# dash-robotics/perception

Measured on AMD Instinct MI355X. Metric: frames/sec (640x480 D435 cloud, plane+cluster+ICP), higher is better.
Workload: dtype f32

## Files before the change

### perception_amd/csrc/k_icp_lat.hip

```cpp
#include "kernels.hpp"
#include "icp_solve_row.hpp"
#include "lat_search.hpp"

namespace cd {

#ifdef CD_LAT_TIMERS
__device__ unsigned long long g_lat_stats[8];
extern "C" int cd_debug_lat_stats(unsigned long long* out, int reset) {
    if (hipMemcpyFromSymbol(out, HIP_SYMBOL(g_lat_stats), sizeof(g_lat_stats)) != hipSuccess) return -1;
    if (reset) { unsigned long long z[8] = {0}; (void)hipMemcpyToSymbol(HIP_SYMBOL(g_lat_stats), z, sizeof(z)); }
    return 0;
}
#define LAT_T(k) { const long long tn_ = clock64(); tph[k] += tn_ - tlast; tlast = tn_; }
#else
#define LAT_T(k)
#endif

struct LatSlot {
    int k, src_off, n, tslot;
    int phase;
    int gen;
    int ready;
    int pad;
};
enum { LAT_ITER = 0, LAT_FIT = 1, LAT_EMPTY = 2 };

#ifndef CD_LAT_SOLVE_ROW
#define CD_LAT_SOLVE_ROW 1
#endif
#ifndef CD_LAT_WAVES_PER_EU
#define CD_LAT_WAVES_PER_EU 4
#endif
template <int CPW, int WPC, bool BOUNDED>
__global__ void __launch_bounds__(CPW * WPC * WAVE, CD_LAT_WAVES_PER_EU)
k_icp_lat(int nitems, const int* __restrict__ order, const IcpCluster* __restrict__ cl, IcpState* __restrict__ st,
          unsigned long long* __restrict__ accf, const IcpLattice* __restrict__ lats, float4* __restrict__ src,
          const float4* __restrict__ src0, int* __restrict__ queue, unsigned long long* __restrict__ busy,
          unsigned long long* __restrict__ busy_out, IcpParams prm, IcpBound bnd) {
    __shared__ float4 s_tab[CPW][LAT_MAX_TAB];
    __shared__ int4 s_face[CPW][2 * LAT_MAX_FACES];
    __shared__ unsigned long long s_acc[CPW][16];
    __shared__ IcpState s_so[CPW];
    __shared__ LatSlot s_slot[CPW];
    __shared__ int s_flags[2];
    __shared__ unsigned s_nv[BOUNDED ? CPW : 1];
    const int lane = threadIdx.x & 63, wave = threadIdx.x >> 6;
    const int slot = wave / WPC, sub = wave % WPC;
    const long long wg_t0 = wall_clock64();
    auto refill = [&](int s) {
        LatSlot& sl = s_slot[s];
        for (int i = 0; i < 16; ++i) s_acc[s][i] = 0ull;
        if constexpr (BOUNDED) s_nv[s] = 0u;
        sl.ready = 0;
        for (;;) {
            const int item = atomicAdd(queue, 1);
            if (item >= nitems) { sl.phase = LAT_EMPTY; return; }
            const int k = order[item];
            if (st[2 * (size_t)k].done) continue;
            const IcpCluster c = cl[k];
            sl.k = k; sl.src_off = c.src_off; sl.n = c.n; sl.tslot = c.slot;
            s_so[s] = st[2 * (size_t)k];
            sl.phase = LAT_ITER;
            sl.gen += 1;
            return;
        }
    };
    if (threadIdx.x < CPW) { s_slot[threadIdx.x].gen = 0; refill(threadIdx.x); }
    if (threadIdx.x == 0) { s_flags[0] = 0; s_flags[1] = 1; }
    __syncthreads();
    int my_gen = 0;
#ifdef CD_LAT_TIMERS
    long long tph[6] = {0, 0, 0, 0, 0, 0}, tlast = clock64();
#endif
    for (;;) {
        if (s_flags[1]) {
            const LatSlot sl = s_slot[slot];
            const bool mine = sl.phase != LAT_EMPTY && sl.gen != my_gen;
            if (mine) {
                const IcpLattice* __restrict__ L = lats + sl.tslot;
                for (int i = sub * WAVE + lane; i < L->ntab; i += WPC * WAVE) s_tab[slot][i] = L->tab[i];
                if (sub == 0 && lane < LAT_MAX_FACES) {
                    const int f = lane, w = L->w[f], u = L->fast[f], v = 3 - w - u;
                    s_face[slot][f] = make_int4(w, u, L->base[f], __float_as_int(L->c[f]));
                    s_face[slot][LAT_MAX_FACES + f] = make_int4(L->toff[u], L->toff[v < 0 || v > 2 ? 0 : v], L->n[u], 0);
                }
                my_gen = sl.gen;
            }
            __syncthreads();
        }
        LAT_T(5)
        {
            const int phase = __builtin_amdgcn_readfirstlane(s_slot[slot].phase), n = __builtin_amdgcn_readfirstlane(s_slot[slot].n);
            const int src_off = __builtin_amdgcn_readfirstlane(s_slot[slot].src_off), tslot = __builtin_amdgcn_readfirstlane(s_slot[slot].tslot);
            const int npass = (n + 63) >> 6;
            float4* pts = src + src_off;
            const float4* tab = s_tab[slot];
            const int4* face = s_face[slot];
            LatFaces F;
            {
                const IcpLattice* __restrict__ L = lats + (phase == LAT_EMPTY ? 0 : tslot);
                lat_faces_load(L, F);
            }
            const bool nf3 = F.nface <= 3;
            if (phase == LAT_ITER) {
                const bool moved = s_so[slot].iters > 0;
                float T[12];
#pragma unroll
                for (int i = 0; i < 12; ++i) T[i] = s_so[slot].T[i];
                unsigned long long S[16];
#pragma unroll
                for (int i = 0; i < 16; ++i) S[i] = 0ull;
                unsigned nv = 0u;
                float4 pnext = pts[min((sub << 6) + lane, n - 1)];
                for (int pss = sub; pss < npass; pss += WPC) {
                    const int myq = (pss << 6) + lane;
                    const bool act = myq < n;
                    const float4 p = pnext;
                    pnext = pts[min(((pss + WPC) << 6) + lane, n - 1)];
                    float px = p.x, py = p.y, pz = p.z;
                    if (moved) {
                        xform(T, p.x, p.y, p.z, px, py, pz);
                        if (act) pts[myq] = make_float4(px, py, pz, p.w);
                    }
                    const LatHit h = F.axes ? lat_nearest_axes<true>(tab, face, F, px, py, pz)
                                            : (nf3 ? lat_nearest<true, 3>(tab, face, F, px, py, pz) : lat_nearest<true, LAT_MAX_FACES>(tab, face, F, px, py, pz));
                    const bool keep = act && (!BOUNDED || h.d <= bnd.d2_max);
                    if constexpr (BOUNDED) nv += (unsigned)__popcll(ballot64(keep));
                    if (keep) {
                        const float pv[3] = {px, py, pz}, qv[3] = {h.nx, h.ny, h.nz};
                        const float big_c = fmaxf(fmaxf(fmaxf(fabsf(px), fabsf(py)), fabsf(pz)), fmaxf(fmaxf(fabsf(h.nx), fabsf(h.ny)), fabsf(h.nz)));
                        if (big_c < 256.f && h.d < 16384.f) {
#pragma unroll
                            for (int a = 0; a < 3; ++a) {
                                S[a] += LatFix<FIX_SHIFT>::bits(pv[a]);
                                S[3 + a] += LatFix<FIX_SHIFT>::bits(qv[a]);
#pragma unroll
                                for (int b = 0; b < 3; ++b) S[6 + 3 * a + b] += LatFix<FIX_SHIFT>::bits(__fmul_rn(qv[a], pv[b]));
                            }
                            S[15] += LatFix<FIX_SHIFT_D2>::bits(h.d);
                        } else {
#pragma unroll
                            for (int a = 0; a < 3; ++a) {
                                S[a] += (unsigned long long)fixq(pv[a], FIX_SHIFT) + LatFix<FIX_SHIFT>::C;
                                S[3 + a] += (unsigned long long)fixq(qv[a], FIX_SHIFT) + LatFix<FIX_SHIFT>::C;
#pragma unroll
                                for (int b = 0; b < 3; ++b) S[6 + 3 * a + b] += (unsigned long long)fixq(__fmul_rn(qv[a], pv[b]), FIX_SHIFT) + LatFix<FIX_SHIFT>::C;
                            }
                            S[15] += (unsigned long long)fixq(h.d, FIX_SHIFT_D2) + LatFix<FIX_SHIFT_D2>::C;
                        }
                    }
                }
                if (sub < npass) wave_fold_to_lds(S, 16, s_acc[slot]);
                if constexpr (BOUNDED) { if (sub < npass && lane == 0) atomicAdd(&s_nv[slot], nv); }
                if (sub == 0 && lane == 0) s_slot[slot].ready = 1;
            } else if (phase == LAT_FIT) {
                const float4* pts0 = src0 + src_off;
                float T[12], Tf[12];
#pragma unroll
                for (int i = 0; i < 12; ++i) {
                    T[i] = __int_as_float(__builtin_amdgcn_readfirstlane(__float_as_int(s_so[slot].T[i])));
                    Tf[i] = __int_as_float(__builtin_amdgcn_readfirstlane(__float_as_int(s_so[slot].Tfinal[i])));
                }
                unsigned long long S[16];
#pragma unroll
                for (int i = 0; i < 16; ++i) S[i] = 0ull;
                float4 pnext = pts[min((sub << 6) + lane, n - 1)], p0next = pts0[min((sub << 6) + lane, n - 1)];
                for (int pss = sub; pss < npass; pss += WPC) {
                    const int myq = (pss << 6) + lane;
                    const bool act = myq < n;
                    const float4 p = pnext, p0 = p0next;
                    pnext = pts[min(((pss + WPC) << 6) + lane, n - 1)];
                    p0next = pts0[min(((pss + WPC) << 6) + lane, n - 1)];
                    float ox, oy, oz;
                    xform(T, p.x, p.y, p.z, ox, oy, oz);
                    if (act) pts[myq] = make_float4(ox, oy, oz, p.w);
                    float qx, qy, qz;
                    xform(Tf, p0.x, p0.y, p0.z, qx, qy, qz);
                    const LatHit h = F.axes ? lat_nearest_axes<false>(tab, face, F, qx, qy, qz)
                                            : (nf3 ? lat_nearest<false, 3>(tab, face, F, qx, qy, qz) : lat_nearest<false, LAT_MAX_FACES>(tab, face, F, qx, qy, qz));
                    if (act) S[0] += h.d < 16384.f ? LatFix<FIX_SHIFT_D2>::bits(h.d) : (unsigned long long)fixq(h.d, FIX_SHIFT_D2) + LatFix<FIX_SHIFT_D2>::C;
                }
                if (sub < npass) wave_fold_to_lds(S, 1, s_acc[slot]);
            }
        }
        LAT_T(0)
        if (threadIdx.x == 0) s_flags[1] = 0;
        __syncthreads();
        LAT_T(1)
#if CD_LAT_SOLVE_ROW
        const int tid = (int)threadIdx.x | s_flags[0];
        if (tid < CPW * 16) {
            const int s = tid >> 4, l = tid & 15;
            LatSlot& sl = s_slot[s];
            const int phase = sl.phase, ready = sl.ready;
            const int nv = BOUNDED && phase == LAT_ITER ? (int)s_nv[s] : sl.n;
            const unsigned long long off = (unsigned long long)nv * LatFix<FIX_SHIFT>::C, off_d = (unsigned long long)nv * LatFix<FIX_SHIFT_D2>::C;
            if (phase == LAT_ITER && ready) {
                RowLanes row(tid);
                RowLanes::V<unsigned long long> a;
                a.v = s_acc[s][l] - (l == 15 ? off_d : off);
                const int done = icp_step_row<BOUNDED>(row, s_so[s], a, nv, prm);
                s_acc[s][l] = 0ull;
                if (l == 0) {
                    if (done) sl.phase = LAT_FIT;
                    if constexpr (BOUNDED) s_nv[s] = 0u;
                    sl.ready = 0;
                }
            } else if (phase == LAT_FIT && l == 0) {
                s_so[s].done = 1;
                st[2 * (size_t)sl.k] = s_so[s];
                st[2 * (size_t)sl.k + 1] = s_so[s];
                accf[sl.k] = s_acc[s][0] - off_d;
                refill(s);
                if (sl.phase != LAT_EMPTY) s_flags[1] = 1;
            }
        }
#else
        if (threadIdx.x < CPW) {
            const int s = threadIdx.x;
            LatSlot& sl = s_slot[s];
            const int nv = BOUNDED && sl.phase == LAT_ITER ? (int)s_nv[s] : sl.n;
            const unsigned long long off = (unsigned long long)nv * LatFix<FIX_SHIFT>::C, off_d = (unsigned long long)nv * LatFix<FIX_SHIFT_D2>::C;
            if (sl.phase == LAT_ITER && sl.ready) {
                for (int i = 0; i < 15; ++i) s_acc[s][i] -= off;
                s_acc[s][15] -= off_d;
                if (icp_step<BOUNDED>(s_so[s], s_acc[s], nv, prm)) sl.phase = LAT_FIT;
                for (int i = 0; i < 16; ++i) s_acc[s][i] = 0ull;
                if constexpr (BOUNDED) s_nv[s] = 0u;
                sl.ready = 0;
            } else if (sl.phase == LAT_FIT) {
                s_so[s].done = 1;
                st[2 * (size_t)sl.k] = s_so[s];
                st[2 * (size_t)sl.k + 1] = s_so[s];
                accf[sl.k] = s_acc[s][0] - off_d;
                refill(s);
                if (sl.phase != LAT_EMPTY) s_flags[1] = 1;
            }
        }
#endif
        LAT_T(2)
        __syncthreads();
        LAT_T(3)
#ifdef CD_LAT_TIMERS
        tph[4] += 1;
#endif
        int all_empty = 1;
#pragma unroll
        for (int s = 0; s < CPW; ++s) all_empty &= s_slot[s].phase == LAT_EMPTY ? 1 : 0;
        if (all_empty) break;
    }
#ifdef CD_LAT_TIMERS
    if (threadIdx.x == 0) for (int i = 0; i < 6; ++i) atomicAdd(&g_lat_stats[i], (unsigned long long)tph[i]);
#endif
    if (threadIdx.x == 0 && busy) {
        atomicAdd(busy, (unsigned long long)(wall_clock64() - wg_t0) * (unsigned long long)(CPW * WPC));
        if (busy_out) {
            __threadfence();
            if (atomicAdd(queue + 1, 1) == (int)gridDim.x - 1) {
                __threadfence();
                *busy_out = atomicAdd(busy, 0ull);
            }
        }
    }
}

__device__ __forceinline__ bool lat_same_bits(float a, float b) { return __float_as_uint(a) == __float_as_uint(b); }

__global__ void __launch_bounds__(BLOCK) k_lat_nn(const IcpLattice* __restrict__ L, const float4* __restrict__ q, int n, int* __restrict__ out_idx,
                                                  float* __restrict__ out_d2) {
    __shared__ float4 s_tab[LAT_MAX_TAB];
    __shared__ int4 s_face[2 * LAT_MAX_FACES];
    LatFaces F;
    lat_stage<BLOCK>(L, F, s_tab, s_face);
    for (int base = blockIdx.x * BLOCK; base < n; base += gridDim.x * BLOCK) {
        const int i = base + threadIdx.x;
        const float4 p = q[i < n ? i : n - 1];
        const LatHit h = lat_nearest<true, LAT_MAX_FACES, true>(s_tab, s_face, F, p.x, p.y, p.z);
        const LatHit g = lat_nearest<false, 3>(s_tab, s_face, F, p.x, p.y, p.z);
        bool same = F.nface > 3 || h.d == g.d;
        const int idx = lat_index(s_face, F, h);
        if (F.axes) {
            const LatHit a = lat_nearest_axes<true, true>(s_tab, s_face, F, p.x, p.y, p.z);
            const LatHit b = lat_nearest_axes<false>(s_tab, s_face, F, p.x, p.y, p.z);
            same = same && a.d == h.d && b.d == h.d && lat_same_bits(a.nx, h.nx) && lat_same_bits(a.ny, h.ny) && lat_same_bits(a.nz, h.nz) &&
                   lat_index(s_face, F, a) == idx;
        }
        if (i < n) { out_idx[i] = idx; out_d2[i] = same ? h.d : __uint_as_float(0x7fc00000u); }
    }
}

template <int CPW, int WPC>
static void launch_lat_shape(hipStream_t s, int nitems, int n_wg, const int* order, const IcpCluster* cl, IcpState* st, unsigned long long* accf,
                             const IcpLattice* lats, float4* src, const float4* src0, int* queue, unsigned long long* busy, unsigned long long* busy_out,
                             IcpParams prm, const IcpBound& bnd) {
    if (bnd.bounded)
        hipLaunchKernelGGL((k_icp_lat<CPW, WPC, true>), dim3(n_wg), dim3(CPW * WPC * WAVE), 0, s, nitems, order, cl, st, accf, lats, src, src0, queue, busy, busy_out, prm, bnd);
    else
        hipLaunchKernelGGL((k_icp_lat<CPW, WPC, false>), dim3(n_wg), dim3(CPW * WPC * WAVE), 0, s, nitems, order, cl, st, accf, lats, src, src0, queue, busy, busy_out, prm, bnd);
}
void launch_icp_lat(hipStream_t s, int nitems, int cpw, int wpc, int n_wg, const IcpProblems& P, const IcpTemplates& T, const IcpScratch& S,
                    unsigned long long* busy, unsigned long long* busy_out, IcpParams prm, const IcpBound& bnd) {
    if (nitems <= 0 || n_wg <= 0) return;
#define CD_LAT_CASE(C, W) if (cpw == C && wpc == W) return launch_lat_shape<C, W>(s, nitems, n_wg, P.order, P.cl, P.st, P.accf, T.lats, S.src, S.src0, S.queue, busy, busy_out, prm, bnd);
    CD_LAT_CASE(1, 1) CD_LAT_CASE(1, 2) CD_LAT_CASE(1, 4) CD_LAT_CASE(1, 8) CD_LAT_CASE(1, 16)
    CD_LAT_CASE(2, 1) CD_LAT_CASE(2, 2) CD_LAT_CASE(2, 4)
    CD_LAT_CASE(4, 1) CD_LAT_CASE(4, 2) CD_LAT_CASE(4, 4)
    CD_LAT_CASE(8, 1) CD_LAT_CASE(8, 2)
#undef CD_LAT_CASE
    launch_lat_shape<1, 4>(s, nitems, n_wg, P.order, P.cl, P.st, P.accf, T.lats, S.src, S.src0, S.queue, busy, busy_out, prm, bnd);
}
void launch_lat_nn(hipStream_t s, const IcpLattice* lat, const float4* q, int n, int* out_idx, float* out_d2) {
    if (n <= 0) return;
    const int g = (n + BLOCK - 1) / BLOCK;
    hipLaunchKernelGGL(k_lat_nn, dim3(g < 1024 ? g : 1024), dim3(BLOCK), 0, s, lat, q, n, out_idx, out_d2);
}

}
```

Baseline: 209,500.

## Replace wave reduction of moment sums with DPP row-transpose fold

Replaces the generic wave_fold_to_lds reduction of the 16 fixed-point 64-bit moment sums with a transpose-style fold. Half the lanes swap registers, and DPP adds within a row halve the live sums at each step, so each lane of a 16-lane row ends up holding one distinct sum. permlane16/32 swaps then combine the rows, and each of the first 16 lanes does one LDS atomic. The __syncthreads after the per-slot work is also swapped for a raw lgkmcnt wait plus s_barrier, which skips waiting on outstanding global memory ops. It adds timer probes and a host-side check of the fold, and it relies on hand-written asm DPP and gfx950 permlane intrinsics.

```diff
diff --git a/perception_amd/csrc/k_icp_lat.hip b/perception_amd/csrc/k_icp_lat.hip
--- a/perception_amd/csrc/k_icp_lat.hip
+++ b/perception_amd/csrc/k_icp_lat.hip
@@ -1,19 +1,24 @@
 #include "kernels.hpp"
 #include "icp_solve_row.hpp"
 #include "lat_search.hpp"
+#include "lat_fold.hpp"
 
 namespace cd {
 
 #ifdef CD_LAT_TIMERS
-__device__ unsigned long long g_lat_stats[8];
+__device__ unsigned long long g_lat_stats[16];
 extern "C" int cd_debug_lat_stats(unsigned long long* out, int reset) {
     if (hipMemcpyFromSymbol(out, HIP_SYMBOL(g_lat_stats), sizeof(g_lat_stats)) != hipSuccess) return -1;
-    if (reset) { unsigned long long z[8] = {0}; (void)hipMemcpyToSymbol(HIP_SYMBOL(g_lat_stats), z, sizeof(z)); }
+    if (reset) { unsigned long long z[16] = {0}; (void)hipMemcpyToSymbol(HIP_SYMBOL(g_lat_stats), z, sizeof(z)); }
     return 0;
 }
-#define LAT_T(k) { const long long tn_ = clock64(); tph[k] += tn_ - tlast; tlast = tn_; }
+#define LAT_T(k) { const long long tn_ = clock64(); tph[k] += tn_ - tlast; tlast = tn_; tsub = tn_; }
+#define LAT_S(k) { const long long tn_ = clock64(); tph[k] += tn_ - tsub; tsub = tn_; }
+#define LAT_VM() asm volatile("s_waitcnt vmcnt(0)" ::: "memory");
 #else
 #define LAT_T(k)
+#define LAT_S(k)
+#define LAT_VM()
 #endif
 
 struct LatSlot {
@@ -31,6 +36,8 @@
 #ifndef CD_LAT_WAVES_PER_EU
 #define CD_LAT_WAVES_PER_EU 4
 #endif
+__device__ __forceinline__ void lds_barrier() { asm volatile("s_waitcnt lgkmcnt(0)\n\ts_barrier" ::: "memory"); }
+
 template <int CPW, int WPC, bool BOUNDED>
 __global__ void __launch_bounds__(CPW * WPC * WAVE, CD_LAT_WAVES_PER_EU)
 k_icp_lat(int nitems, const int* __restrict__ order, const IcpCluster* __restrict__ cl, IcpState* __restrict__ st,
@@ -70,7 +77,7 @@
     __syncthreads();
     int my_gen = 0;
 #ifdef CD_LAT_TIMERS
-    long long tph[6] = {0, 0, 0, 0, 0, 0}, tlast = clock64();
+    long long tph[10] = {0, 0, 0, 0, 0, 0, 0, 0, 0, 0}, tlast = clock64(), tsub = tlast;
 #endif
     for (;;) {
         if (s_flags[1]) {
@@ -112,6 +119,7 @@
                 for (int i = 0; i < 16; ++i) S[i] = 0ull;
                 unsigned nv = 0u;
                 float4 pnext = pts[min((sub << 6) + lane, n - 1)];
+                LAT_VM() LAT_S(6)
                 for (int pss = sub; pss < npass; pss += WPC) {
                     const int myq = (pss << 6) + lane;
                     const bool act = myq < n;
@@ -150,9 +158,11 @@
                         }
                     }
                 }
-                if (sub < npass) wave_fold_to_lds(S, 16, s_acc[slot]);
+                LAT_S(7)
+                if (sub < npass) wave_fold_rows_to_lds<16>(S, s_acc[slot]);
                 if constexpr (BOUNDED) { if (sub < npass && lane == 0) atomicAdd(&s_nv[slot], nv); }
                 if (sub == 0 && lane == 0) s_slot[slot].ready = 1;
+                LAT_S(8)
             } else if (phase == LAT_FIT) {
                 const float4* pts0 = src0 + src_off;
                 float T[12], Tf[12];
@@ -165,6 +175,7 @@
 #pragma unroll
                 for (int i = 0; i < 16; ++i) S[i] = 0ull;
                 float4 pnext = pts[min((sub << 6) + lane, n - 1)], p0next = pts0[min((sub << 6) + lane, n - 1)];
+                LAT_VM() LAT_S(6)
                 for (int pss = sub; pss < npass; pss += WPC) {
                     const int myq = (pss << 6) + lane;
                     const bool act = myq < n;
@@ -180,12 +191,14 @@
                                             : (nf3 ? lat_nearest<false, 3>(tab, face, F, qx, qy, qz) : lat_nearest<false, LAT_MAX_FACES>(tab, face, F, qx, qy, qz));
                     if (act) S[0] += h.d < 16384.f ? LatFix<FIX_SHIFT_D2>::bits(h.d) : (unsigned long long)fixq(h.d, FIX_SHIFT_D2) + LatFix<FIX_SHIFT_D2>::C;
                 }
-                if (sub < npass) wave_fold_to_lds(S, 1, s_acc[slot]);
+                LAT_S(7)
+                if (sub < npass) wave_fold_rows_to_lds<1>(S, s_acc[slot]);
+                LAT_S(8)
             }
         }
         LAT_T(0)
         if (threadIdx.x == 0) s_flags[1] = 0;
-        __syncthreads();
+        lds_barrier();
         LAT_T(1)
 #if CD_LAT_SOLVE_ROW
         const int tid = (int)threadIdx.x | s_flags[0];
@@ -250,7 +263,7 @@
         if (all_empty) break;
     }
 #ifdef CD_LAT_TIMERS
-    if (threadIdx.x == 0) for (int i = 0; i < 6; ++i) atomicAdd(&g_lat_stats[i], (unsigned long long)tph[i]);
+    if (threadIdx.x == 0) for (int i = 0; i < 10; ++i) atomicAdd(&g_lat_stats[i], (unsigned long long)tph[i]);
 #endif
     if (threadIdx.x == 0 && busy) {
         atomicAdd(busy, (unsigned long long)(wall_clock64() - wg_t0) * (unsigned long long)(CPW * WPC));
diff --git a/perception_amd/csrc/lat_fold.hpp b/perception_amd/csrc/lat_fold.hpp
--- /dev/null
+++ b/perception_amd/csrc/lat_fold.hpp
@@ -0,0 +1,104 @@
+#pragma once
+
+#ifdef __HIPCC__
+#define CD_FOLD_FN __device__ __forceinline__
+#else
+#define CD_FOLD_FN inline
+#endif
+
+namespace cd {
+
+enum { LANE_X8 = 8, LANE_X7 = 7, LANE_X2 = 2, LANE_X1 = 1 };
+
+template <int NSUM, class W>
+CD_FOLD_FN void wave_fold_rows(W& w, typename W::template V<unsigned long long> (&A)[16], unsigned long long* dst) {
+    static_assert(NSUM == 16 || NSUM == 1, "the fold of 16 moment sums or of the one fitness sum");
+    if constexpr (NSUM == 16) {
+        w.template swap_if<8>(8, A, A + 8);
+        w.template add_from<LANE_X8, 8>(A, A + 8);
+        w.template swap_if<4>(4, A, A + 4);
+        w.template add_from<LANE_X7, 4>(A, A + 4);
+        w.template swap_if<2>(2, A, A + 2);
+        w.template add_from<LANE_X2, 2>(A, A + 2);
+        w.template swap_if<1>(1, A, A + 1);
+        w.template add_from<LANE_X1, 1>(A, A + 1);
+    } else {
+        w.template add_from<LANE_X8, 1>(A, A);
+        w.template add_from<LANE_X7, 1>(A, A);
+        w.template add_from<LANE_X2, 1>(A, A);
+        w.template add_from<LANE_X1, 1>(A, A);
+    }
+    w.sum_rows(A[0]);
+    w.each([&](int l) { if (l < NSUM) w.add_to(dst + l, A[0](l)); });
+}
+
+#ifdef __HIPCC__
+struct WaveLanes {
+    template <class T>
+    struct V {
+        T v;
+        __device__ __forceinline__ T& operator()(int) { return v; }
+        __device__ __forceinline__ const T& operator()(int) const { return v; }
+    };
+    using U64 = V<unsigned long long>;
+    int lane;
+    __device__ __forceinline__ explicit WaveLanes(int thread) : lane(thread & 63) {}
+    template <class F> __device__ __forceinline__ void each(F&& f) { f(lane); }
+    template <int N> __device__ __forceinline__ void swap_if(int bit, U64* a, U64* b) const {
+        if (lane & bit) {
+#pragma unroll
+            for (int i = 0; i < N; ++i) {
+                unsigned alo = (unsigned)a[i].v, ahi = (unsigned)(a[i].v >> 32), blo = (unsigned)b[i].v, bhi = (unsigned)(b[i].v >> 32);
+                asm volatile("v_swap_b32 %0, %1" : "+v"(alo), "+v"(blo));
+                asm volatile("v_swap_b32 %0, %1" : "+v"(ahi), "+v"(bhi));
+                a[i].v = ((unsigned long long)ahi << 32) | alo;
+                b[i].v = ((unsigned long long)bhi << 32) | blo;
+            }
+        }
+    }
+#define CD_FOLD_ADD(ctrl)                                                                            \
+    "v_add_co_u32_dpp %0, vcc, %2, %0 " ctrl " row_mask:0xf bank_mask:0xf bound_ctrl:0\n\t"          \
+    "v_addc_co_u32_dpp %1, vcc, %3, %1, vcc " ctrl " row_mask:0xf bank_mask:0xf bound_ctrl:0"
+    template <int P> static __device__ __forceinline__ void add1(U64& a, const U64& b) {
+        unsigned alo = (unsigned)a.v, ahi = (unsigned)(a.v >> 32);
+        const unsigned blo = (unsigned)b.v, bhi = (unsigned)(b.v >> 32);
+        if constexpr (P == LANE_X8) asm volatile("s_nop 1\n\t" CD_FOLD_ADD("row_ror:8") : "+v"(alo), "+v"(ahi) : "v"(blo), "v"(bhi) : "vcc");
+        else if constexpr (P == LANE_X7) asm volatile("s_nop 1\n\t" CD_FOLD_ADD("row_half_mirror") : "+v"(alo), "+v"(ahi) : "v"(blo), "v"(bhi) : "vcc");
+        else if constexpr (P == LANE_X2) asm volatile("s_nop 1\n\t" CD_FOLD_ADD("quad_perm:[2,3,0,1]") : "+v"(alo), "+v"(ahi) : "v"(blo), "v"(bhi) : "vcc");
+        else asm volatile("s_nop 1\n\t" CD_FOLD_ADD("quad_perm:[1,0,3,2]") : "+v"(alo), "+v"(ahi) : "v"(blo), "v"(bhi) : "vcc");
+        a.v = ((unsigned long long)ahi << 32) | alo;
+    }
+#undef CD_FOLD_ADD
+    template <int P, int N> __device__ __forceinline__ void add_from(U64* a, const U64* b) const {
+        static_assert(P == LANE_X8 || P == LANE_X7 || P == LANE_X2 || P == LANE_X1, "a partner inside the row");
+#pragma unroll
+        for (int i = 0; i < N; ++i) add1<P>(a[i], b[i]);
+    }
+    __device__ __forceinline__ void sum_rows(U64& a) const {
+#ifdef __HIP_DEVICE_COMPILE__
+        {
+            const unsigned lo = (unsigned)a.v, hi = (unsigned)(a.v >> 32);
+            const auto rl = __builtin_amdgcn_permlane16_swap(lo, lo, false, false), rh = __builtin_amdgcn_permlane16_swap(hi, hi, false, false);
+            a.v = (((unsigned long long)rh[0] << 32) | rl[0]) + (((unsigned long long)rh[1] << 32) | rl[1]);
+        }
+        {
+            const unsigned lo = (unsigned)a.v, hi = (unsigned)(a.v >> 32);
+            const auto rl = __builtin_amdgcn_permlane32_swap(lo, lo, false, false), rh = __builtin_amdgcn_permlane32_swap(hi, hi, false, false);
+            a.v = (((unsigned long long)rh[0] << 32) | rl[0]) + (((unsigned long long)rh[1] << 32) | rl[1]);
+        }
+#endif
+    }
+    __device__ __forceinline__ void add_to(unsigned long long* dst, unsigned long long v) const { atomicAdd(dst, v); }
+};
+
+template <int NSUM>
+__device__ __forceinline__ void wave_fold_rows_to_lds(const unsigned long long (&S)[16], unsigned long long* dst) {
+    WaveLanes w((int)threadIdx.x);
+    WaveLanes::U64 A[16];
+#pragma unroll
+    for (int i = 0; i < (NSUM == 16 ? 16 : 1); ++i) A[i].v = S[i];
+    wave_fold_rows<NSUM>(w, A, dst);
+}
+#endif
+
+}
diff --git a/perception_amd/csrc/lat_fold_check.cpp b/perception_amd/csrc/lat_fold_check.cpp
--- /dev/null
+++ b/perception_amd/csrc/lat_fold_check.cpp
@@ -0,0 +1,113 @@
+#include <cstdint>
+#include <cstdio>
+#include <cstdlib>
+#include <cstring>
+#include <initializer_list>
+
+#include "lat_fold.hpp"
+
+namespace {
+
+struct HostWave {
+    template <class T>
+    struct V {
+        T v[64];
+        T& operator()(int l) { return v[l]; }
+        const T& operator()(int l) const { return v[l]; }
+    };
+    using U64 = V<unsigned long long>;
+    unsigned long long* base = nullptr;
+    int nsum = 0, adds = 0;
+    unsigned seen = 0;
+    bool bad = false;
+    int cur = -1;
+    template <class F> void each(F&& f) { for (cur = 0; cur < 64; ++cur) f(cur); cur = -1; }
+    template <int N> void swap_if(int bit, U64* a, U64* b) const {
+        for (int l = 0; l < 64; ++l)
+            if (l & bit)
+                for (int i = 0; i < N; ++i) { const unsigned long long t = a[i].v[l]; a[i].v[l] = b[i].v[l]; b[i].v[l] = t; }
+    }
+    template <int P, int N> void add_from(U64* a, const U64* b) const {
+        static_assert(P == cd::LANE_X8 || P == cd::LANE_X7 || P == cd::LANE_X2 || P == cd::LANE_X1, "a partner inside the row");
+        for (int i = 0; i < N; ++i) {
+            unsigned long long r[64];
+            for (int l = 0; l < 64; ++l) r[l] = a[i].v[l] + b[i].v[l ^ P];
+            std::memcpy(a[i].v, r, sizeof(r));
+        }
+    }
+    void sum_rows(U64& a) const {
+        unsigned long long r[64];
+        for (int l = 0; l < 64; ++l) r[l] = a.v[l & 15] + a.v[(l & 15) + 16] + a.v[(l & 15) + 32] + a.v[(l & 15) + 48];
+        std::memcpy(a.v, r, sizeof(r));
+    }
+    void add_to(unsigned long long* dst, unsigned long long v) {
+        const long k = dst - base;
+        if (cur < 0 || cur >= nsum || k != cur || (seen >> cur & 1u)) bad = true;
+        else { seen |= 1u << cur; *dst += v; }
+        ++adds;
+    }
+};
+
+struct Rng {
+    uint64_t s;
+    uint64_t next() {
+        uint64_t z = (s += 0x9E3779B97F4A7C15ull);
+        z = (z ^ (z >> 30)) * 0xBF58476D1CE4E5B9ull;
+        z = (z ^ (z >> 27)) * 0x94D049BB133111EBull;
+        return z ^ (z >> 31);
+    }
+};
+
+unsigned long long value(Rng& g, int kind, int lane, int sum) {
+    switch (kind) {
+        case 0: return g.next();
+        case 1: return 0xFFFFFFFFull - (g.next() & 0xFFull);
+        case 2: return ~0ull;
+        case 3: return (g.next() & 63) == (unsigned)lane ? g.next() : 0ull;
+        case 4: return sum == (int)(g.s & 15) ? g.next() : 0ull;
+        default: return (g.next() & 0xFFFFFFFFull) | 0x80000000ull;
+    }
+}
+
+template <int NSUM>
+long run(Rng& g, int kind, int waves) {
+    unsigned long long dst[16], want[16];
+    for (int i = 0; i < 16; ++i) dst[i] = want[i] = g.next();
+    for (int wv = 0; wv < waves; ++wv) {
+        static HostWave::U64 A[16];
+        unsigned long long tot[16] = {0};
+        for (int i = 0; i < 16; ++i)
+            for (int l = 0; l < 64; ++l) {
+                A[i].v[l] = i < NSUM ? value(g, kind, l, i) : 0xDEADBEEFCAFEF00Dull;
+                tot[i] += A[i].v[l];
+            }
+        HostWave w;
+        w.base = dst;
+        w.nsum = NSUM;
+        cd::wave_fold_rows<NSUM>(w, A, dst);
+        if (w.bad || w.adds != NSUM || w.seen != (NSUM == 16 ? 0xFFFFu : 1u)) { std::printf("wrong lanes add: kind %d adds %d seen %x\n", kind, w.adds, w.seen); return -1; }
+        for (int i = 0; i < NSUM; ++i) want[i] += tot[i];
+        for (int l = 0; l < 64; ++l)
+            if (A[0].v[l] != tot[NSUM == 16 ? (l & 15) : 0]) { std::printf("lane %d does not hold its sum: kind %d\n", l, kind); return -1; }
+    }
+    for (int i = 0; i < 16; ++i)
+        if (dst[i] != want[i]) { std::printf("sum %d differs: kind %d waves %d NSUM %d\n", i, kind, waves, NSUM); return -1; }
+    return waves;
+}
+
+}
+
+int main(int argc, char** argv) {
+    const int rounds = argc > 1 ? std::atoi(argv[1]) : 200;
+    Rng g{0x1234567ull};
+    long n = 0;
+    for (int r = 0; r < rounds; ++r)
+        for (int kind = 0; kind < 6; ++kind)
+            for (int waves : {1, 2, 3, 8, 16}) {
+                const long a = run<16>(g, kind, waves), b = run<1>(g, kind, waves);
+                if (a < 0 || b < 0) return 1;
+                n += a + b;
+            }
+    std::printf("ok %ld\n", n);
+    return 0;
+}
```

Measured after the change: 210,300, median of 6. About the same (+0.4%).
